# ecmwf/anemoi-transform

Measured on AMD Instinct MI355X. Metric: grid-points/sec regridded, O1280->0.25deg x137 levels, higher is better.
Workload: dtype f64; 1 GPU; O1280 (6599680 pts) -> 0.25 deg lat-lon (1038240 pts), k=4 inverse-distance regrid x 137 levels per stack; layout=columns, target_order=natural (row-major)

## Files before the change

### anemoi-transform_amd/csrc/atx_regrid_fields.inc

```

namespace atx {

template <typename T, int K, bool WEIGHTED, bool EPI, bool PAD>
__global__ void __launch_bounds__(kBlock)
regrid_fields_ell_kernel(const T* __restrict__ src, T* __restrict__ out,
                         const int32_t* __restrict__ idx, const T* __restrict__ w,
                         int64_t n_tgt, int k_rt, int n_lev, int64_t src_pitch, int64_t out_pitch,
                         int lev_chunk, unsigned n_tiles,
                         const atx_level_op* __restrict__ prog, int n_stage,
                         const uint8_t* __restrict__ tgt_mask) {
    const int k = K > 0 ? K : k_rt;
    const unsigned tile_id = xcd_tile(blockIdx.x, n_tiles);
    const int64_t t = (int64_t)tile_id * kBlock + threadIdx.x;
    if (t >= n_tgt) return;
    const int l0 = blockIdx.y * lev_chunk;
    const int l1 = min(n_lev, l0 + lev_chunk);
    const bool masked = (EPI && tgt_mask) ? (tgt_mask[t] != 0) : false;

    if (K > 0) {
        int64_t p[K > 0 ? K : 1];
        T wj[K > 0 ? K : 1];
        bool present[K > 0 ? K : 1];
#pragma unroll
        for (int j = 0; j < (K > 0 ? K : 1); ++j) {
            p[j] = idx[t * K + j];
            wj[j] = WEIGHTED ? w[t * K + j] : T(1);
            present[j] = !PAD || p[j] >= 0;
        }
        if (PAD) {
            const int64_t spare = present[0] ? p[0] : 0;
#pragma unroll
            for (int j = 0; j < (K > 0 ? K : 1); ++j)
                if (!present[j]) p[j] = spare;
        }
#pragma unroll 4
        for (int l = l0; l < l1; ++l) {
            const T* s = src + (int64_t)l * src_pitch;
            T acc;
            if (WEIGHTED) {
                T sv[K > 0 ? K : 1];
#pragma unroll
                for (int j = 0; j < (K > 0 ? K : 1); ++j) sv[j] = s[p[j]];
                acc = T(0);
#pragma unroll
                for (int j = 0; j < (K > 0 ? K : 1); ++j) {
                    const T sum = acc + wj[j] * sv[j];
                    acc = present[j] ? sum : acc;
                }
            } else {
                acc = s[p[0]];
            }
            if (EPI) {
                for (int st = 0; st < n_stage; ++st)
                    acc = apply_level_op(load_level_op<T>(prog, (int64_t)st * n_lev + l), acc, masked);
            }
            out[(int64_t)l * out_pitch + t] = acc;
        }
    } else {
        constexpr int LC = 16;
        for (int lc = l0; lc < l1; lc += LC) {
            const int nl = min(LC, l1 - lc);
            const T* s0 = src + (int64_t)lc * src_pitch;
            T acc[LC];
#pragma unroll
            for (int i = 0; i < LC; ++i) acc[i] = T(0);
            for (int j = 0; j < k; ++j) {
                const T wv = WEIGHTED ? w[t * k + j] : T(1);
                const int64_t pj = idx[t * k + j];
                if (PAD && pj < 0) continue;
#pragma unroll
                for (int i = 0; i < LC; ++i)
                    if (i < nl) acc[i] = acc[i] + wv * s0[(int64_t)i * src_pitch + pj];
            }
#pragma unroll
            for (int i = 0; i < LC; ++i) {
                if (i < nl) {
                    T v = acc[i];
                    if (EPI) {
                        for (int st = 0; st < n_stage; ++st)
                            v = apply_level_op(load_level_op<T>(prog, (int64_t)st * n_lev + lc + i), v, masked);
                    }
                    out[(int64_t)(lc + i) * out_pitch + t] = v;
                }
            }
        }
    }
}

template <typename T, bool EPI, int R>
__global__ void __launch_bounds__(kBlock)
regrid_fields_csr_head_kernel(const T* __restrict__ src, T* __restrict__ out,
                              const int32_t* __restrict__ indptr, const int32_t* __restrict__ indices,
                              const T* __restrict__ data, int64_t n_tgt, int n_lev,
                              int64_t src_pitch, int64_t out_pitch, int lev_chunk, unsigned n_tiles,
                              const atx_level_op* __restrict__ prog, int n_stage,
                              const uint8_t* __restrict__ tgt_mask) {
    const unsigned tile_id = xcd_tile(blockIdx.x, n_tiles);
    const int64_t t = (int64_t)tile_id * kBlock + threadIdx.x;
    if (t >= n_tgt) return;
    const int l0 = blockIdx.y * lev_chunk;
    const int l1 = min(n_lev, l0 + lev_chunk);
    const int64_t j0 = indptr[t], j1 = indptr[t + 1];
    const bool masked = (EPI && tgt_mask) ? (tgt_mask[t] != 0) : false;
    int64_t p[R];
    T wj[R];
    bool present[R];
#pragma unroll
    for (int j = 0; j < R; ++j) {
        present[j] = j0 + j < j1;
        p[j] = present[j] ? (int64_t)indices[j0 + j] : (j > 0 ? p[0] : 0);
        wj[j] = present[j] ? data[j0 + j] : T(0);
    }
    const int64_t rest = j0 + R;
#pragma unroll 4
    for (int l = l0; l < l1; ++l) {
        const T* s = src + (int64_t)l * src_pitch;
        T sv[R];
#pragma unroll
        for (int j = 0; j < R; ++j) sv[j] = s[p[j]];
        T acc = T(0);
#pragma unroll
        for (int j = 0; j < R; ++j) {
            const T sum = acc + wj[j] * sv[j];
            acc = present[j] ? sum : acc;
        }
        for (int64_t jj = rest; jj < j1; ++jj) acc = acc + data[jj] * s[indices[jj]];
        if (EPI) {
            for (int st = 0; st < n_stage; ++st)
                acc = apply_level_op(load_level_op<T>(prog, (int64_t)st * n_lev + l), acc, masked);
        }
        out[(int64_t)l * out_pitch + t] = acc;
    }
}

constexpr int kFieldsChunk = 16;
template <typename T, bool EPI>
__global__ void __launch_bounds__(kBlock)
regrid_fields_csr_kernel(const T* __restrict__ src, T* __restrict__ out,
                         const int32_t* __restrict__ indptr, const int32_t* __restrict__ indices,
                         const T* __restrict__ data, int64_t n_tgt, int n_lev,
                         int64_t src_pitch, int64_t out_pitch, unsigned n_tiles,
                         const atx_level_op* __restrict__ prog, int n_stage,
                         const uint8_t* __restrict__ tgt_mask) {
    const unsigned tile_id = xcd_tile(blockIdx.x, n_tiles);
    const int64_t t = (int64_t)tile_id * kBlock + threadIdx.x;
    if (t >= n_tgt) return;
    const int l0 = blockIdx.y * kFieldsChunk;
    const int nl = min(kFieldsChunk, n_lev - l0);
    const int64_t j0 = indptr[t], j1 = indptr[t + 1];
    const T* s0 = src + (int64_t)l0 * src_pitch;
    T acc[kFieldsChunk];
#pragma unroll
    for (int i = 0; i < kFieldsChunk; ++i) acc[i] = T(0);
    for (int64_t jj = j0; jj < j1; ++jj) {
        const int64_t p = indices[jj];
        const T wv = data[jj];
#pragma unroll
        for (int i = 0; i < kFieldsChunk; ++i)
            if (i < nl) acc[i] = acc[i] + wv * s0[(int64_t)i * src_pitch + p];
    }
    const bool masked = (EPI && tgt_mask) ? (tgt_mask[t] != 0) : false;
#pragma unroll
    for (int i = 0; i < kFieldsChunk; ++i) {
        if (i < nl) {
            T v = acc[i];
            if (EPI) {
                for (int st = 0; st < n_stage; ++st)
                    v = apply_level_op(load_level_op<T>(prog, (int64_t)st * n_lev + l0 + i), v, masked);
            }
            out[(int64_t)(l0 + i) * out_pitch + t] = v;
        }
    }
}

template <typename T, int K, bool WEIGHTED, bool PAD = false>
static int launch_fields_ell(const T* src, T* out, const int32_t* idx, const T* w, int64_t n_tgt, int k,
                             int n_lev, int64_t sp, int64_t op, const atx_level_op* prog, int n_stage,
                             const uint8_t* m, hipStream_t st) {
    const unsigned n_tiles = (unsigned)((n_tgt + kBlock - 1) / kBlock);
    const int lev_chunk = pick_lev_chunk(n_lev);
    const unsigned n_chunks = (unsigned)((n_lev + lev_chunk - 1) / lev_chunk);
    ATX_REQUIRE(n_chunks <= 65535, ATX_ENOTIMPL, "regrid_ell: too many level chunks (%u)", n_chunks);
    with_flag(prog != nullptr, [&](auto fused) {
        hipLaunchKernelGGL((regrid_fields_ell_kernel<T, K, WEIGHTED, decltype(fused)::value, PAD>), dim3(n_tiles, n_chunks), dim3(kBlock), 0, st,
                           src, out, idx, w, n_tgt, k, n_lev, sp, op, lev_chunk, n_tiles, prog, n_stage, m);
    });
    ATX_LAUNCH_CHECK("regrid_fields_ell");
    return ATX_OK;
}

template <typename T>
static int dispatch_fields_ell(const T* src, T* out, const int32_t* idx, const T* w, int64_t n_tgt, int k,
                               int n_lev, int64_t sp, int64_t op, bool pad, const atx_level_op* prog, int n_stage,
                               const uint8_t* m, hipStream_t st) {
    if (!w) return launch_fields_ell<T, 1, false>(src, out, idx, w, n_tgt, k, n_lev, sp, op, prog, n_stage, m, st);
    return with_flag(pad, [&](auto padded) {
        constexpr bool PAD = decltype(padded)::value;
        constexpr int kMin = PAD ? 3 : 1;
        auto fixed = [&](auto kc) {
            constexpr int K = decltype(kc)::value >= kMin ? decltype(kc)::value : 0;
            return launch_fields_ell<T, K, true, PAD>(src, out, idx, w, n_tgt, k, n_lev, sp, op, prog, n_stage, m, st);
        };
        switch (k) {
            case 1: return fixed(IntTag<1>{});
            case 2: return fixed(IntTag<2>{});
            case 3: return fixed(IntTag<3>{});
            case 4: return fixed(IntTag<4>{});
            default: return fixed(IntTag<0>{});
        }
    });
}

template <typename T>
static int regrid_fields_ell(const EllBatch& batch, const int32_t* idx, const T* w, int64_t n_tgt, int k, int n_lev, int64_t sp, int64_t op,
                             bool pad, const Epilogue& e, hipStream_t st) {
    for (int i = 0; i < batch.n; ++i) {
        const int rc = dispatch_fields_ell<T>(static_cast<const T*>(batch.src[i]), static_cast<T*>(batch.out[i]), idx, w, n_tgt, k,
                                              n_lev, sp, op, pad, e.prog, e.n_stage, e.mask, st);
        if (rc != ATX_OK) return rc;
    }
    return ATX_OK;
}

template <typename T>
static int regrid_fields_csr(const T* src, T* out, const int32_t* indptr, const int32_t* indices, const T* data, int64_t n_tgt, int64_t nnz,
                             int n_lev, int64_t sp, int64_t op, const atx_level_op* prog, int n_stage, const uint8_t* m, const int32_t* rows,
                             hipStream_t st) {
    ATX_REQUIRE(!rows, ATX_ENOTIMPL, "regrid_csr: an ordered traversal (tgt_rows) is available for ATX_COLUMNS stacks only");
    const unsigned n_tiles = (unsigned)((n_tgt + kBlock - 1) / kBlock);
    const double mean = n_tgt > 0 ? (double)nnz / (double)n_tgt : 0.0;
    if (mean <= 8.0) {
        const int lev_chunk = pick_lev_chunk(n_lev);
        const unsigned chunks = (unsigned)((n_lev + lev_chunk - 1) / lev_chunk);
        ATX_REQUIRE(chunks <= 65535, ATX_ENOTIMPL, "regrid_csr: too many level chunks (%u)", chunks);
        with_flag(prog != nullptr, [&](auto fused) {
            with_flag(mean <= 4.0, [&](auto four) {
                hipLaunchKernelGGL((regrid_fields_csr_head_kernel<T, decltype(fused)::value, decltype(four)::value ? 4 : 8>), dim3(n_tiles, chunks),
                                   dim3(kBlock), 0, st, src, out, indptr, indices, data, n_tgt, n_lev, sp, op, lev_chunk, n_tiles, prog, n_stage, m);
            });
        });
        ATX_LAUNCH_CHECK("regrid_fields_csr_head");
        return ATX_OK;
    }
    const unsigned n_chunks = (unsigned)((n_lev + kFieldsChunk - 1) / kFieldsChunk);
    ATX_REQUIRE(n_chunks <= 65535, ATX_ENOTIMPL, "regrid_csr: too many level chunks (%u)", n_chunks);
    with_flag(prog != nullptr, [&](auto fused) {
        hipLaunchKernelGGL((regrid_fields_csr_kernel<T, decltype(fused)::value>), dim3(n_tiles, n_chunks), dim3(kBlock), 0, st, src, out, indptr, indices,
                           data, n_tgt, n_lev, sp, op, n_tiles, prog, n_stage, m);
    });
    ATX_LAUNCH_CHECK("regrid_fields_csr");
    return ATX_OK;
}

}
```

Baseline: 169.9 billion grid-points/s.

## Stage per-tile source index runs in LDS with double-buffered level loads

Adds a staged ELL regrid kernel. Each block first builds a bitmap of the source index ranges its targets touch, merges them into a few contiguous runs, then streams those runs into shared memory level by level with vectorized coalesced loads, double-buffered across levels. The gathers then read from LDS instead of scattered global memory. It also retunes the level chunking so there are enough groups. The cost is setup atomics, syncs and 48KB of LDS per block (which can lower occupancy), plus a fallback to the direct path when the runs are too sparse or too large.

```diff
diff --git a/anemoi-transform_amd/csrc/atx_fields_runs.hpp b/anemoi-transform_amd/csrc/atx_fields_runs.hpp
--- /dev/null
+++ b/anemoi-transform_amd/csrc/atx_fields_runs.hpp
@@ -0,0 +1,66 @@
+#ifndef ATX_FIELDS_RUNS_HPP
+#define ATX_FIELDS_RUNS_HPP
+
+#include <cstdint>
+
+#if defined(__HIPCC__)
+#define ATX_RUNS_FN __host__ __device__ inline
+#else
+#define ATX_RUNS_FN inline
+#endif
+
+namespace atx {
+
+constexpr int kRunBucketShift = 5;
+constexpr int kRunBucket = 1 << kRunBucketShift;
+constexpr int kRunWords = 64;
+constexpr int kRunSpan = kRunWords * 32 * kRunBucket;
+constexpr int kTileRuns = 6;
+
+ATX_RUNS_FN int runs_from_bitmap(const uint32_t* bits, int n_words, int* first, int* last) {
+    int n = 0;
+    bool open = false;
+    for (int i = 0; i < n_words; ++i) {
+        const uint32_t w = bits[i];
+        int pos = 0;
+        while (pos < 32) {
+            const uint32_t rest = w >> pos;
+            if (!open) {
+                if (rest == 0) break;
+                pos += __builtin_ctz(rest);
+                if (n == kTileRuns) return -1;
+                first[n] = i * 32 + pos;
+                open = true;
+            } else {
+                const uint32_t zeros = ~rest;
+                if (zeros == 0) break;
+                pos += __builtin_ctz(zeros);
+                if (pos >= 32) break;
+                last[n++] = i * 32 + pos - 1;
+                open = false;
+            }
+        }
+    }
+    if (open) last[n++] = n_words * 32 - 1;
+    return n;
+}
+
+ATX_RUNS_FN int run_of_bucket(int b, const int* last, int n) {
+    int r = 0;
+    while (r + 1 < n && b > last[r]) ++r;
+    return r;
+}
+
+ATX_RUNS_FN int layout_runs(const int* lo, const int* hi, int n, int vec, int* start, int* base) {
+    int total = 0;
+    for (int r = 0; r < n; ++r) {
+        start[r] = lo[r] / vec * vec;
+        base[r] = total;
+        total += (hi[r] - start[r] + vec) / vec * vec;
+    }
+    return total;
+}
+
+}
+
+#endif
diff --git a/anemoi-transform_amd/csrc/atx_regrid_fields.inc b/anemoi-transform_amd/csrc/atx_regrid_fields.inc
--- a/anemoi-transform_amd/csrc/atx_regrid_fields.inc
+++ b/anemoi-transform_amd/csrc/atx_regrid_fields.inc
@@ -1,5 +1,37 @@
+
+#include "atx_fields_runs.hpp"
 
 namespace atx {
+
+template <typename T, int K, bool WEIGHTED, bool EPI>
+__device__ __forceinline__ void fields_ell_direct_levels(const T* __restrict__ src, T* __restrict__ out, const int64_t (&p)[K], const T (&wj)[K],
+                                                         const bool (&present)[K], int64_t t, bool live, int l0, int l1, int n_lev,
+                                                         int64_t src_pitch, int64_t out_pitch, const atx_level_op* __restrict__ prog,
+                                                         int n_stage, bool masked) {
+#pragma unroll 4
+    for (int l = l0; l < l1; ++l) {
+        const T* s = src + (int64_t)l * src_pitch;
+        T acc;
+        if (WEIGHTED) {
+            T sv[K];
+#pragma unroll
+            for (int j = 0; j < K; ++j) sv[j] = s[p[j]];
+            acc = T(0);
+#pragma unroll
+            for (int j = 0; j < K; ++j) {
+                const T sum = acc + wj[j] * sv[j];
+                acc = present[j] ? sum : acc;
+            }
+        } else {
+            acc = s[p[0]];
+        }
+        if (EPI) {
+            for (int st = 0; st < n_stage; ++st)
+                acc = apply_level_op(load_level_op<T>(prog, (int64_t)st * n_lev + l), acc, masked);
+        }
+        if (live) out[(int64_t)l * out_pitch + t] = acc;
+    }
+}
 
 template <typename T, int K, bool WEIGHTED, bool EPI, bool PAD>
 __global__ void __launch_bounds__(kBlock)
@@ -33,29 +65,8 @@
             for (int j = 0; j < (K > 0 ? K : 1); ++j)
                 if (!present[j]) p[j] = spare;
         }
-#pragma unroll 4
-        for (int l = l0; l < l1; ++l) {
-            const T* s = src + (int64_t)l * src_pitch;
-            T acc;
-            if (WEIGHTED) {
-                T sv[K > 0 ? K : 1];
-#pragma unroll
-                for (int j = 0; j < (K > 0 ? K : 1); ++j) sv[j] = s[p[j]];
-                acc = T(0);
-#pragma unroll
-                for (int j = 0; j < (K > 0 ? K : 1); ++j) {
-                    const T sum = acc + wj[j] * sv[j];
-                    acc = present[j] ? sum : acc;
-                }
-            } else {
-                acc = s[p[0]];
-            }
-            if (EPI) {
-                for (int st = 0; st < n_stage; ++st)
-                    acc = apply_level_op(load_level_op<T>(prog, (int64_t)st * n_lev + l), acc, masked);
-            }
-            out[(int64_t)l * out_pitch + t] = acc;
-        }
+        fields_ell_direct_levels<T, (K > 0 ? K : 1), WEIGHTED, EPI>(src, out, p, wj, present, t, true, l0, l1, n_lev, src_pitch, out_pitch, prog,
+                                                                    n_stage, masked);
     } else {
         constexpr int LC = 16;
         for (int lc = l0; lc < l1; lc += LC) {
@@ -84,6 +95,182 @@
                 }
             }
         }
+    }
+}
+
+constexpr int kStageBytes = 24 * 1024;
+constexpr int kStageWaste = 8;
+
+struct FieldsRunScratch {
+    uint32_t bits[kRunWords];
+    int first[kTileRuns], last[kTileRuns];
+    int lo[kTileRuns], hi[kTileRuns];
+    int start[kTileRuns], base[kTileRuns];
+    int min_idx, max_idx, entries, n_runs, total;
+};
+
+template <typename T, int K, bool WEIGHTED, bool EPI, bool PAD>
+__global__ void __launch_bounds__(kBlock)
+regrid_fields_ell_staged_kernel(const T* __restrict__ src, T* __restrict__ out,
+                                const int32_t* __restrict__ idx, const T* __restrict__ w,
+                                int64_t n_tgt, int n_lev, int64_t src_pitch, int64_t out_pitch,
+                                int lev_chunk, unsigned n_tiles,
+                                const atx_level_op* __restrict__ prog, int n_stage,
+                                const uint8_t* __restrict__ tgt_mask) {
+    constexpr int VEC = Vec16<T>::N;
+    constexpr int kElems = kStageBytes / (int)sizeof(T);
+    constexpr int kSlots = kElems / VEC / kBlock;
+    using V = typename NativeVec<T, VEC>::type;
+    __shared__ V stage[2][kElems / VEC];
+    __shared__ FieldsRunScratch rs;
+
+    const int tid = threadIdx.x;
+    const unsigned tile_id = xcd_tile(blockIdx.x, n_tiles);
+    const int64_t t = (int64_t)tile_id * kBlock + tid;
+    const bool live = t < n_tgt;
+    const int l0 = blockIdx.y * lev_chunk;
+    const int l1 = min(n_lev, l0 + lev_chunk);
+    const bool masked = (EPI && tgt_mask && live) ? (tgt_mask[t] != 0) : false;
+
+    int64_t p[K];
+    T wj[K];
+    bool present[K];
+#pragma unroll
+    for (int j = 0; j < K; ++j) {
+        p[j] = live ? (int64_t)idx[t * K + j] : (int64_t)-1;
+        wj[j] = (WEIGHTED && live) ? w[t * K + j] : T(1);
+        present[j] = live && (!PAD || p[j] >= 0);
+    }
+
+    if (tid < kRunWords) rs.bits[tid] = 0;
+    if (tid < kTileRuns) {
+        rs.lo[tid] = INT32_MAX;
+        rs.hi[tid] = -1;
+    }
+    if (tid == 0) {
+        rs.min_idx = INT32_MAX;
+        rs.max_idx = -1;
+        rs.entries = 0;
+    }
+    __syncthreads();
+    {
+        int mn = INT32_MAX, mx = -1, cnt = 0;
+#pragma unroll
+        for (int j = 0; j < K; ++j) {
+            if (present[j]) {
+                mn = min(mn, (int)p[j]);
+                mx = max(mx, (int)p[j]);
+                ++cnt;
+            }
+        }
+        if (cnt > 0) {
+            atomicMin(&rs.min_idx, mn);
+            atomicMax(&rs.max_idx, mx);
+            atomicAdd(&rs.entries, cnt);
+        }
+    }
+    __syncthreads();
+    const int origin = rs.min_idx & ~(kRunBucket - 1);
+    bool staged = rs.max_idx >= 0 && rs.max_idx - origin < kRunSpan;
+    int bucket[K];
+    if (staged) {
+#pragma unroll
+        for (int j = 0; j < K; ++j) {
+            bucket[j] = present[j] ? ((int)p[j] - origin) >> kRunBucketShift : 0;
+            if (present[j]) atomicOr(&rs.bits[bucket[j] >> 5], 1u << (bucket[j] & 31));
+        }
+    }
+    __syncthreads();
+    if (staged && tid == 0) rs.n_runs = runs_from_bitmap(rs.bits, kRunWords, rs.first, rs.last);
+    __syncthreads();
+    staged = staged && rs.n_runs > 0;
+    int run[K];
+    if (staged) {
+        const int n = rs.n_runs;
+#pragma unroll
+        for (int j = 0; j < K; ++j) {
+            run[j] = present[j] ? run_of_bucket(bucket[j], rs.last, n) : 0;
+            if (present[j]) {
+                atomicMin(&rs.lo[run[j]], (int)p[j]);
+                atomicMax(&rs.hi[run[j]], (int)p[j]);
+            }
+        }
+    }
+    __syncthreads();
+    if (staged && tid == 0) rs.total = layout_runs(rs.lo, rs.hi, rs.n_runs, VEC, rs.start, rs.base);
+    __syncthreads();
+    staged = staged && rs.total <= kElems && rs.total <= kStageWaste * rs.entries;
+
+    if (!staged) {
+        if (!live) return;
+        const int64_t spare = present[0] ? p[0] : 0;
+#pragma unroll
+        for (int j = 0; j < K; ++j)
+            if (!present[j]) p[j] = spare;
+        fields_ell_direct_levels<T, K, WEIGHTED, EPI>(src, out, p, wj, present, t, true, l0, l1, n_lev, src_pitch, out_pitch, prog, n_stage, masked);
+        return;
+    }
+
+    int q[K];
+#pragma unroll
+    for (int j = 0; j < K; ++j) q[j] = present[j] ? rs.base[run[j]] + ((int)p[j] - rs.start[run[j]]) : 0;
+#pragma unroll
+    for (int j = 1; j < K; ++j)
+        if (!present[j]) q[j] = q[0];
+    int from[kSlots];
+    {
+        const int n = rs.n_runs, total = rs.total;
+#pragma unroll
+        for (int i = 0; i < kSlots; ++i) {
+            const int e = (tid + i * kBlock) * VEC;
+            int r = 0;
+            while (r + 1 < n && e >= rs.base[r + 1]) ++r;
+            from[i] = e < total ? rs.start[r] + (e - rs.base[r]) : -1;
+        }
+    }
+
+    V regs[kSlots];
+    auto fetch = [&](int l) {
+        const T* s = src + (int64_t)l * src_pitch;
+#pragma unroll
+        for (int i = 0; i < kSlots; ++i)
+            if (from[i] >= 0) regs[i] = *reinterpret_cast<const V*>(s + from[i]);
+    };
+    auto put = [&](int b) {
+#pragma unroll
+        for (int i = 0; i < kSlots; ++i)
+            if (from[i] >= 0) stage[b][tid + i * kBlock] = regs[i];
+    };
+    fetch(l0);
+    put(0);
+    __syncthreads();
+    int cur = 0;
+    for (int l = l0; l < l1; ++l) {
+        const bool more = l + 1 < l1;
+        if (more) fetch(l + 1);
+        const T* sb = reinterpret_cast<const T*>(stage[cur]);
+        T acc;
+        if (WEIGHTED) {
+            T sv[K];
+#pragma unroll
+            for (int j = 0; j < K; ++j) sv[j] = sb[q[j]];
+            acc = T(0);
+#pragma unroll
+            for (int j = 0; j < K; ++j) {
+                const T sum = acc + wj[j] * sv[j];
+                acc = present[j] ? sum : acc;
+            }
+        } else {
+            acc = sb[q[0]];
+        }
+        if (EPI) {
+            for (int st = 0; st < n_stage; ++st)
+                acc = apply_level_op(load_level_op<T>(prog, (int64_t)st * n_lev + l), acc, masked);
+        }
+        if (live) out[(int64_t)l * out_pitch + t] = acc;
+        if (more) put(cur ^ 1);
+        __syncthreads();
+        cur ^= 1;
     }
 }
 
@@ -178,9 +365,23 @@
                              int n_lev, int64_t sp, int64_t op, const atx_level_op* prog, int n_stage,
                              const uint8_t* m, hipStream_t st) {
     const unsigned n_tiles = (unsigned)((n_tgt + kBlock - 1) / kBlock);
-    const int lev_chunk = pick_lev_chunk(n_lev);
-    const unsigned n_chunks = (unsigned)((n_lev + lev_chunk - 1) / lev_chunk);
+    int lev_chunk = pick_lev_chunk(n_lev);
+    unsigned n_chunks = (unsigned)((n_lev + lev_chunk - 1) / lev_chunk);
     ATX_REQUIRE(n_chunks <= 65535, ATX_ENOTIMPL, "regrid_ell: too many level chunks (%u)", n_chunks);
+    if constexpr (K > 0) {
+        if (aligned16(src) && sp % Vec16<T>::N == 0) {
+            constexpr unsigned kStagedMinGroups = 1536;
+            const unsigned want = std::min(n_chunks, (kStagedMinGroups + n_tiles - 1) / std::max(n_tiles, 1u));
+            lev_chunk = (n_lev + (int)want - 1) / (int)std::max(want, 1u);
+            n_chunks = (unsigned)((n_lev + lev_chunk - 1) / lev_chunk);
+            with_flag(prog != nullptr, [&](auto fused) {
+                hipLaunchKernelGGL((regrid_fields_ell_staged_kernel<T, K, WEIGHTED, decltype(fused)::value, PAD>), dim3(n_tiles, n_chunks), dim3(kBlock), 0,
+                                   st, src, out, idx, w, n_tgt, n_lev, sp, op, lev_chunk, n_tiles, prog, n_stage, m);
+            });
+            ATX_LAUNCH_CHECK("regrid_fields_ell_staged");
+            return ATX_OK;
+        }
+    }
     with_flag(prog != nullptr, [&](auto fused) {
         hipLaunchKernelGGL((regrid_fields_ell_kernel<T, K, WEIGHTED, decltype(fused)::value, PAD>), dim3(n_tiles, n_chunks), dim3(kBlock), 0, st,
                            src, out, idx, w, n_tgt, k, n_lev, sp, op, lev_chunk, n_tiles, prog, n_stage, m);
```

Result: no change. 169.9 billion grid-points/s (-0.0%).
